# MartinMikkelsen/TensorTrainNumerics.jl

Hardware: AMD Instinct MI355X
Metric: TT cores/sec for QTT Laplacian apply+round, d=30 rank-64 (higher is better)
Workload: dtype f64

## Files before the change

### tensortrainnumerics.jl_amd/csrc/ttn_dense_kernels.h

```cpp
#pragma once
#include "ttn_wg_prims.h"
#include "ttn_wg_gemm.h"
#include "ttn_wg_lq.h"
#include "ttn_wg_jacobi.h"
#include "ttn_wg_chol.h"

struct CompressArgs {
    TTDev tt;
    long long max_bond;
    double truncerr;
    int sweeps;
    int k_single;
    int k_first, k_last;
    double* scratch;
    long long scratch_stride;
    int pmax, qmax;
    double* sv_out;
    int sv_steps;
    int* status;
    int* sweep_stats;
    int fast;
    int fused;
    TTODev op;
    TTDev x;
    int rank_rule;
    int fused_first_real;
    int* next_train;
};

#define COMPRESS_LDS_X_DOUBLES (128 * 128)
#define COMPRESS_LDS_BYTES ((GEMM_LDS_TOTAL + 32 + 2 * QR_NB * QR_NB + QR_NB + 8 + 8 + 128) * sizeof(double))
#define FAST_KAPPA_MAX 128.0
#define FAST_KAPPA_POLISH 32768.0
#define FAST_POLISH_DROP 1.0e-12
#define FAST_DIAG_TOL 2.0e-12
#define FAST_CHECK_TOL 2.0e-11

struct BondCtx {
    double *ldsX, *red, *Ts, *Ss, *taus, *scal, *nrm2;
    int* iflag;
    double *M, *M2, *Vb, *Wb, *Us, *Xg, *sig, *sigs, *Ga, *Gb, *Cc, *T1, *T2, *T3;
    int* perm;
};

#define CHOLQR_PIVOT_MAX 1.0e11
#define CHOLQR_ORTH_MAX 1.0e-3
#define CHOLQR_CHECK_TOL 1.0e-9

__device__ __noinline__ double wg_img_load(double* img, int row_off, const double* src, int p, double* red) {
    img = unip(img); src = unip(src); p = uni32(p); row_off = uni32(row_off); red = unip(red);
    lds_f64* X = (lds_f64*)img;
    double dev = 0.0;
    wg_batched<8>((long long)p * p, [&](long long e) { const int ei = (int)e; return src[ei % p + 128 * (ei / p)]; },
                  [&](long long e, double v) {
                      const int ei = (int)e, i = ei % p, j = ei / p;
                      X[row_off + i + 128 * j] = v;
                      dev = fmax(dev, fabs(v - ((i == j) ? 1.0 : 0.0)));
                  });
    return unif64(wg_max(dev, red));
}

__device__ __noinline__ void wg_trsm_lower_cols(int p, int q, const double* img, const double* M, long long ldm, double s_, double* Q, long long ldq) {
    p = uni32(p); q = uni32(q); img = unip(img); M = unip(M); Q = unip(Q); ldm = uni64(ldm); ldq = uni64(ldq); s_ = unif64(s_);
    const lds_f64* L = (const lds_f64*)img;
    gmem_f64* Mg = (gmem_f64*)M;
    gmem_wf64* Qg = (gmem_wf64*)Q;
    for (int c = threadIdx.x; c < q; c += TTN_WG) {
        for (int i0 = 0; i0 < p; i0 += 16) {
            const int nb = (p - i0 < 16) ? p - i0 : 16;
            double v[16];
#pragma unroll
            for (int ii = 0; ii < 16; ++ii) v[ii] = Mg[(long long)(i0 + (ii < nb ? ii : 0)) * ldm + c];
#pragma unroll
            for (int ii = 0; ii < 16; ++ii) v[ii] *= s_;
            for (int j0 = 0; j0 < i0; j0 += 16) {
                double qv[16];
#pragma unroll
                for (int jj = 0; jj < 16; ++jj) qv[jj] = Qg[(long long)(j0 + jj) * ldq + c];
#pragma unroll
                for (int jj = 0; jj < 16; ++jj)
#pragma unroll
                    for (int ii = 0; ii < 16; ++ii) v[ii] = fma(-L[(j0 + jj) * 128 + i0 + ii], qv[jj], v[ii]);
            }
#pragma unroll
            for (int k = 0; k < 16; ++k) {
                if (k < nb) {
                    v[k] = v[k] / L[(i0 + k) * 128 + i0 + k];
#pragma unroll
                    for (int ii = k + 1; ii < 16; ++ii) v[ii] = fma(-L[(i0 + k) * 128 + i0 + ii], v[k], v[ii]);
                }
            }
#pragma unroll
            for (int ii = 0; ii < 16; ++ii) if (ii < nb) Qg[(long long)(i0 + ii) * ldq + c] = v[ii];
        }
    }
    __syncthreads();
}

__device__ __noinline__ void wg_tril_mul_lds(int p, double* img) {
    p = uni32(p); img = unip(img);
    lds_f64* X = (lds_f64*)img;
    constexpr int NE = (64 * 64 + TTN_WG - 1) / TTN_WG;
    double acc[NE];
#pragma unroll
    for (int u = 0; u < NE; ++u) {
        const int e = threadIdx.x + u * TTN_WG, i = e % p, j = e / p;
        double a = 0.0;
        if (e < p * p && i >= j)
            for (int k = j; k <= i; ++k) a = fma(X[64 + i + 128 * k], X[k + 128 * j], a);
        acc[u] = a;
    }
    __syncthreads();
    for (int e = threadIdx.x; e < p * 128; e += TTN_WG) X[e] = 0.0;
    __syncthreads();
#pragma unroll
    for (int u = 0; u < NE; ++u) {
        const int e = threadIdx.x + u * TTN_WG, i = e % p, j = e / p;
        if (e < p * p && i >= j) X[i + 128 * j] = acc[u];
    }
    __syncthreads();
}

__device__ __noinline__ void wg_scale_image(const double* X, int ldx, int x_in_lds, const double* sigs, const int* perm, View Lo, double* Us, int p, int r,
                                            double s0, double aneg, int mode, double* tab) {
    X = unip(X); ldx = uni32(ldx); x_in_lds = uni32(x_in_lds); sigs = unip(sigs); perm = unip(perm); Lo = uniView(Lo); Us = unip(Us);
    p = uni32(p); r = uni32(r); s0 = unif64(s0); aneg = unif64(aneg); mode = uni32(mode); tab = unip(tab);
    lds_f64* f1 = (lds_f64*)tab; lds_f64* f2 = f1 + 128;
    lds_i32* pj = (lds_i32*)(f2 + 128); lds_i32* coff = pj + 128; lds_i32* roff = coff + 128;
    const int tid = threadIdx.x, lane = tid & 63, wave = tid >> 6;
    const double sq0 = sqrt(s0);
    for (int j = tid; j < r; j += TTN_WG) {
        const double sj = sigs[j];
        const bool keep = (sj > 0.0) && (sj * sj > aneg);
        double a, b_;
        if (mode == 0) { const double rs = sqrt(sj); a = sq0 / rs; b_ = sq0 / (sj * rs); }
        else if (mode == 1) { a = 1.0 / sj; b_ = s0 / sj; }
        else { a = s0; b_ = 1.0 / (sj * sj); }
        f1[j] = keep ? a : 0.0; f2[j] = keep ? b_ : 0.0;
        pj[j] = perm[j]; coff[j] = (int)ix(Lo.c, j);
    }
    for (int i = tid; i < p; i += TTN_WG) roff[i] = (int)ix(Lo.r, i);
    __syncthreads();
    gmem_wf64* Lg = (gmem_wf64*)Lo.p;
    gmem_wf64* Ug = (gmem_wf64*)Us;
    for (int j = wave; j < r; j += TTN_NWAVES) {
        const double a = f1[j], b_ = f2[j];
        const int c = pj[j], co = coff[j];
        for (int row = lane; row < p; row += 64) {
            const double xv = x_in_lds ? ((const lds_f64*)X)[c * ldx + row] : X[(long long)c * ldx + row];
            Lg[roff[row] + co] = xv * a;
            Ug[j * p + row] = xv * b_;
        }
    }
    __syncthreads();
}

__device__ __noinline__ double wg_check_diag_tab(const double* sigs, const double* D, int ldd, int r, double s0, double* tab, double* red) {
    sigs = unip(sigs); D = unip(D); ldd = uni32(ldd); r = uni32(r); s0 = unif64(s0); tab = unip(tab); red = unip(red);
    lds_f64* t = (lds_f64*)tab; lds_f64* ref = t + 128;
    const int tid = threadIdx.x, lane = tid & 63, wave = tid >> 6;
    for (int i = tid; i < r; i += TTN_WG) { const double si = sigs[i]; t[i] = 1.0 / sqrt(s0 * si); ref[i] = si * s0; }
    __syncthreads();
    gmem_f64* Dg = (gmem_f64*)D;
    double worst = 0.0;
    for (int j = wave; j < r; j += TTN_NWAVES) {
        const double tj = t[j];
        for (int i = lane; i < r; i += 64) {
            const double dv = Dg[i + ldd * j];
            const double dev = fabs(dv - ((i == j) ? ref[i] : 0.0)) * (t[i] * tj);
            worst = fmax(worst, dev);
        }
    }
    return unif64(wg_max(worst, red));
}

__device__ __noinline__ double wg_check_diag_tab2(const double* sigs, const double* D1, const double* D2, int ldd, int r, double s0, double* tab, double* red) {
    sigs = unip(sigs); D1 = unip(D1); D2 = unip(D2); ldd = uni32(ldd); r = uni32(r); s0 = unif64(s0); tab = unip(tab); red = unip(red);
    lds_f64* t = (lds_f64*)tab; lds_f64* ref = t + 128;
    const int tid = threadIdx.x, lane = tid & 63, wave = tid >> 6;
    for (int i = tid; i < r; i += TTN_WG) { const double si = sigs[i]; t[i] = 1.0 / sqrt(s0 * si); ref[i] = si * s0; }
    __syncthreads();
    gmem_f64* D1g = (gmem_f64*)D1; gmem_f64* D2g = (gmem_f64*)D2;
    double worst = 0.0;
    for (int j = wave; j < r; j += TTN_NWAVES) {
        const double tj = t[j];
        for (int i = lane; i < r; i += 64) {
            const double d1 = D1g[i + ldd * j], d2 = D2g[i + ldd * j];
            const double rf = (i == j) ? ref[i] : 0.0, sc = t[i] * tj;
            worst = fmax(worst, fmax(fabs(d1 - rf) * sc, fabs(d2 - rf) * sc));
        }
    }
    return unif64(wg_max(worst, red));
}

__device__ __noinline__ double wg_diag_test_t3(const double* Ga, const double* Gb, double* T3, double* tab, double* red) {
    Ga = unip(Ga); Gb = unip(Gb); T3 = unip(T3); tab = unip(tab); red = unip(red);
    lds_f64* sd = (lds_f64*)tab; lds_f64* isd = sd + 64;
    const int tid = threadIdx.x, lane = tid & 63, wave = tid >> 6;
    gmem_f64* Gag = (gmem_f64*)Ga; gmem_f64* Gbg = (gmem_f64*)Gb; gmem_wf64* Tg = (gmem_wf64*)T3;
    for (int i = tid; i < 64; i += TTN_WG) { const double d = Gag[i * 129]; const double sq = (d > 0.0) ? sqrt(d) : 0.0; sd[i] = sq; isd[i] = (d > 0.0) ? 1.0 / sq : -1.0; }
    __syncthreads();
    double w = 0.0;
    const double si = sd[lane], ii = isd[lane];
    constexpr int NJ = 64 / TTN_NWAVES;
    double ga[NJ], gb[NJ];
#pragma unroll
    for (int u = 0; u < NJ; ++u) { const int j = wave + TTN_NWAVES * u; ga[u] = Gag[lane + 128 * j]; gb[u] = Gbg[lane + 128 * j]; }
#pragma unroll
    for (int u = 0; u < NJ; ++u) {
        const int j = wave + TTN_NWAVES * u;
        const double ij = isd[j];
        if (lane != j) w = fmax(w, (ii > 0.0 && ij > 0.0) ? fabs(ga[u]) * (ii * ij) : 1.0);
        Tg[lane + 128 * j] = si * gb[u] * sd[j];
    }
    w = unif64(wg_max(w, red));
    return w;
}

__device__ __noinline__ void wg_scale_t12_diag(const double* img, const double* sigs, const int* perm, const double* Ga, double* T1, double* T2, int rk,
                                               double fa, double fb, double* tab) {
    img = unip(img); sigs = unip(sigs); perm = unip(perm); Ga = unip(Ga); T1 = unip(T1); T2 = unip(T2); rk = uni32(rk); fa = unif64(fa); fb = unif64(fb); tab = unip(tab);
    lds_f64* c1 = (lds_f64*)tab; lds_f64* c2 = c1 + 64; lds_f64* sd = c2 + 64; lds_f64* isd = sd + 64;
    lds_i32* pj = (lds_i32*)(isd + 64);
    const lds_f64* X = (const lds_f64*)img;
    const int tid = threadIdx.x, lane = tid & 63, wave = tid >> 6;
    for (int j = tid; j < 64; j += TTN_WG) {
        const double d = sqrt(Ga[j * 129]); sd[j] = d; isd[j] = 1.0 / d;
        if (j < rk) { const double sj = sigs[j], rs = sqrt(sj); c1[j] = fa / rs; c2[j] = fb / (sj * rs); pj[j] = perm[j]; }
    }
    __syncthreads();
    gmem_wf64* T1g = (gmem_wf64*)T1; gmem_wf64* T2g = (gmem_wf64*)T2;
    const double sdr = sd[lane], isdr = isd[lane];
    for (int j = wave; j < rk; j += TTN_NWAVES) {
        const double xv = X[pj[j] * 128 + lane];
        T1g[j * 128 + lane] = xv * (c1[j] * isdr);
        T2g[j * 128 + lane] = xv * (sdr * c2[j]);
    }
    __syncthreads();
}

__device__ int wg_svd_cols(const CompressArgs& P, const BondCtx& S, int pj, double* X, int ldx, bool in_lds, int mlen = 0) {
    const int tid = threadIdx.x, lane = tid & 63, wave = tid >> 6, nwaves = TTN_WG >> 6;
    const int nsw = (in_lds && mlen) ? wg_jacobi_lds128(mlen, pj, X, S.nrm2, S.iflag, S.red, S.scal)
                  : in_lds ? wg_jacobi_lds128(pj, pj, X, S.nrm2, S.iflag, S.red, S.scal)
#if TTN_LDS_COLS < 128
                  : (pj <= 128) ? wg_jacobi_blocked128(pj, pj, X, ldx, S.ldsX, S.nrm2, S.iflag, S.red, S.scal)
#endif
                  : (pj <= 256) ? wg_jacobi_blocked256(pj, pj, X, ldx, S.ldsX, S.nrm2, S.iflag, S.red, S.scal)
                                : wg_jacobi_cols(pj, pj, X, ldx, S.iflag, S.red, S.scal);
    for (int c = wave; c < pj; c += nwaves) {
        double a = 0.0;
        for (int r = lane; r < (mlen ? mlen : pj); r += 64) { const double v = X[(long long)c * ldx + r]; a = fma(v, v, a); }
        a = wave_sum(a);
        if (lane == 0) S.sig[c] = sqrt(a);
    }
    __syncthreads();
    for (int c = tid; c < pj; c += TTN_WG) {
        const double sc = S.sig[c];
        int pos = 0;
        for (int j = 0; j < pj; ++j) { const double sj = S.sig[j]; pos += (sj > sc) || (sj == sc && j < c); }
        S.perm[pos] = c;
        S.sigs[pos] = sc;
    }
    __syncthreads();
    return nsw;
}

__device__ __forceinline__ int wg_rank_rule_core(int rank_rule, double truncerr, long long max_bond, const double* sigs, int* iflag, int ns, int plen, double s0) {
    if (threadIdx.x == 0) {
        int r = plen;
        if (rank_rule == 1) {
            if (truncerr > 0.0) {
                r = 0;
                const double thr = truncerr * (sigs[0] * s0);
                for (int i = 0; i < ns; ++i) r += (sigs[i] * s0 > thr) ? 1 : 0;
                if (r < 1) r = 1;
            }
        } else if (truncerr > 0.0) {
            double n2 = 0.0;
            for (int i = 0; i < ns; ++i) { const double s = sigs[i] * s0; n2 = fma(s, s, n2); }
            const double nrm = sqrt(n2);
            double cum = 0.0;
            for (int i = plen; i >= 1; --i) {
                const double s = (i <= ns) ? sigs[i - 1] * s0 : 0.0;
                cum = fma(s, s, cum);
                if (sqrt(cum) > truncerr * nrm) { r = i; break; }
            }
        }
        if ((long long)r > max_bond) r = (int)max_bond;
        iflag[1] = r;
// ... 565 lines not shown
    const int n1 = io.n1, n2 = io.n2;
    const int Dl = io.Dl, rm = io.rm, Dr = io.Dr;
    const int mr = n1 * Dl, mc = n2 * Dr;
    double* ck = io.ck;
    double* ck1 = io.ck1;
    const View Am = mkview(ck, Idx{Dl, (long long)n1, 1}, plain((long long)n1 * Dl));
    const View Bm = mkview(ck1, plain(n2), Idx{n2, 1, (long long)n2 * rm});
    const bool wide = mr <= mc;
    const int p = wide ? mr : mc, q = wide ? mc : mr;
    const View Ap = wide ? Am : tview(Bm);
    const View Bp = wide ? Bm : tview(Am);

    BondCtx S;
    S.ldsX = lds;
    S.red = lds + GEMM_LDS_TOTAL;
    S.Ts = S.red + 32;
    S.Ss = S.Ts + QR_NB * QR_NB;
    S.taus = S.Ss + QR_NB * QR_NB;
    S.scal = S.taus + QR_NB;
    S.iflag = reinterpret_cast<int*>(S.scal + 8);
    S.nrm2 = S.scal + 16;
    double* scr = P.scratch + (long long)blockIdx.x * P.scratch_stride;
    const long long pq = (long long)P.pmax * P.qmax;
    S.M = scr;
    S.M2 = S.M + pq;
    S.Vb = S.M2 + pq;
    S.Wb = S.Vb + (long long)QR_NB * P.qmax;
    S.Us = S.Wb + (long long)P.pmax * QR_NB;
    S.Xg = S.Us + (long long)P.pmax * P.pmax;
    S.sig = S.Xg + (long long)P.pmax * P.pmax;
    S.sigs = S.sig + P.pmax;
    S.perm = reinterpret_cast<int*>(S.sigs + P.pmax);
    S.Ga = S.sigs + 2 * P.pmax;
    S.Gb = S.Ga + 128 * 128;
    S.Cc = S.Gb + 128 * 128;
    S.T1 = S.Cc + 128 * 128;
    S.T2 = S.T1 + 128 * 128;
    S.T3 = S.T2 + 128 * 128;
    if (pq >= 3 * 128 * 128) {
        S.Ga = S.M2; S.Gb = S.M2 + 128 * 128; S.T2 = S.M2 + 2 * 128 * 128;
    }

    bool virt_live = false;
    if (virt) {
        if (wide && rm >= p) virt_live = true;
        else wg_materialize_core(P, b, k + 1);
    }

    const View Lfv = mkview(ck, Idx{Dl, (long long)n1, 1}, plain((long long)n1 * Dl));
    int nsw_total = 0;
    bool done = false;

    if (SWAP == 0 && P.fast && rm < p && rm <= TTN_LDS_COLS && rm >= 2) {
        double sa = 0.0, sb = 0.0;
        sa = wg_absmax(ck, (long long)n1 * Dl * rm, S.red);
        sb = wg_absmax(ck1, (long long)n2 * rm * Dr, S.red);
        bool ok = (sa > 0.0) && (sb > 0.0);
        const double sA = wide ? sa : sb, sB = wide ? sb : sa;
        const double s0 = sA * sB;
        const View Gav = mkview(S.Ga, plain(1), plain(128));
        const View Gbv = mkview(S.Gb, plain(1), plain(128));
        const View Ccv = mkview(S.Cc, plain(1), plain(128));
        bool diagA = false;
        if (ok) {
            wg_syrk2(rm, p, tview(Ap), Gav, 1.0 / (sA * sA), rm, q, Bp, Gbv, 1.0 / (sB * sB), lds);
            if (rm == 64 && !(P.fast & 4) && !(P.fast & 8)) {
                const double wmax = wg_diag_test_t3(S.Ga, S.Gb, S.T3, S.Ss, S.red);
                diagA = wmax <= FAST_DIAG_TOL;
            }
            if (diagA) {
            } else if (rm <= TTN_LDS_COLS / 2) {
                for (int e = tid; e < rm * 128; e += TTN_WG) if ((e & 127) < rm) { S.ldsX[e] = S.Ga[e]; S.ldsX[TTN_LDS_IMG / 2 + e] = S.Gb[e]; }
                __syncthreads();
                ok = wg_chol2_lds128(rm, S.ldsX, S.Ts, S.iflag, S.scal + 1) == 0;
                for (int e = tid; e < rm * 128; e += TTN_WG) if ((e & 127) < rm) { S.Ga[e] = S.ldsX[e]; S.Gb[e] = S.ldsX[TTN_LDS_IMG / 2 + e]; }
                __syncthreads();
            } else {
                for (int e = tid; e < rm * 128; e += TTN_WG) if ((e & 127) < rm) S.ldsX[e] = S.Ga[e];
                __syncthreads();
                ok = wg_chol_lds128(rm, S.ldsX, S.red, S.iflag, S.scal + 1) == 0;
                for (int e = tid; e < rm * 128; e += TTN_WG) if ((e & 127) < rm) S.Ga[e] = S.ldsX[e];
                __syncthreads();
                if (ok) {
                    for (int e = tid; e < rm * 128; e += TTN_WG) if ((e & 127) < rm) S.ldsX[e] = S.Gb[e];
                    __syncthreads();
                    ok = wg_chol_lds128(rm, S.ldsX, S.red, S.iflag, S.scal + 1) == 0;
                    for (int e = tid; e < rm * 128; e += TTN_WG) if ((e & 127) < rm) S.Gb[e] = S.ldsX[e];
                    __syncthreads();
                }
            }
        }
        int r = 0, rk = 0;
        if (ok) {
            int nsw = 1;
            if (diagA) {
                ok = wg_eig64(S.T3, 128, S.T2, 64, 64, S.sigs, lds, reinterpret_cast<int*>(S.Ts), S.Ts + 64) == 0;
                for (int j = tid; j < 64; j += TTN_WG) S.perm[j] = j;
                if (tid == 0) S.scal[0] = 64.0 * DBL_EPSILON * DBL_EPSILON * S.sigs[0] * S.sigs[0];
                __syncthreads();
            } else {
            wg_gemm(rm, rm, rm, tview(Gav), Gbv, Ccv, 1.0, 0.0, lds);
            if (rm == 64 && !(P.fast & 4)) {
                wg_gemm(64, 64, 64, Ccv, tview(Ccv), mkview(S.T3, plain(1), plain(128)), 1.0, 0.0, lds);
                ok = wg_eig64(S.T3, 128, S.T2, 64, 64, S.sigs, lds, reinterpret_cast<int*>(S.Ts), S.Ts + 64) == 0;
                for (int j = tid; j < 64; j += TTN_WG) S.perm[j] = j;
                if (tid == 0) S.scal[0] = 64.0 * DBL_EPSILON * DBL_EPSILON * S.sigs[0] * S.sigs[0];
                __syncthreads();
            } else {
                for (int e = tid; e < rm * 128; e += TTN_WG) { const int c = e >> 7, r_ = e & 127; S.ldsX[e] = (r_ < rm) ? S.Cc[c * 128 + r_] : 0.0; }
// ... 88 lines not shown
        for (int attempt = (SWAP == 0 && P.fast && need_lq && (eig_ok || cholqr_ok || (x_in_lds && !lq_in_lds)) && p >= 2) ? 1 : 2; attempt <= 2 && !done; ++attempt) {
            bool ok = true;
            bool use_eig = false;
            bool cholqr = false;
            double gram_trace = 0.0;
            X = (x_in_lds || attempt == 1) ? S.ldsX : S.Xg;
            ldx = (x_in_lds || attempt == 1) ? 128 : p;
            if (attempt == 1) {
                wg_syrk(p, q, Mv, mkview(S.Ga, plain(1), plain(128)), inv_s0 * inv_s0, lds);
                use_eig = eig_ok;
                if (use_eig) {
                    if (p > 64 && p < 128) {
                        for (int e = tid; e < 128 * 128; e += TTN_WG)
                            if ((e & 127) >= p || (e >> 7) >= p) S.Ga[e] = 0.0;
                        __syncthreads();
                    }
                    const int r0 = (int)P.max_bond;
                    const int nev = (P.truncerr > 0.0 || (P.sv_out && step < P.sv_steps)) ? p : r0;
                    { double t_ = 0.0; for (int i = tid; i < p; i += TTN_WG) t_ += S.Ga[i * 129]; gram_trace = unif64(wg_sum(t_, S.red)); }
                    ok = ((p == 64) ? wg_eig64(S.Ga, 128, S.Gb, r0, nev, S.sigs, lds, reinterpret_cast<int*>(S.Ts), S.Ts + 64)
                                    : wg_eig128(S.Ga, S.Gb, r0, nev, S.sigs, lds, reinterpret_cast<int*>(S.Ts), S.Ts + 64)) == 0;
                    for (int j = tid; j < p; j += TTN_WG) { S.perm[j] = j; if (j >= nev) S.sigs[j] = 0.0; }
                    if (tid == 0) S.scal[0] = (double)p * DBL_EPSILON * DBL_EPSILON * S.sigs[0] * S.sigs[0];
                    __syncthreads();
                } else {
                wg_img_load(S.ldsX, 0, S.Ga, p, S.red);
                ok = wg_chol_lds128(p, S.ldsX, S.red, S.iflag, S.scal + 1) == 0;
                if (ok && (P.truncerr > 0.0 || (long long)p <= P.max_bond)) {
                    if (cholqr_ok) { if (unif64(S.scal[1]) <= CHOLQR_PIVOT_MAX) cholqr = true; else ok = false; }
                    else if (unif64(S.scal[1]) > FAST_KAPPA_MAX * FAST_KAPPA_MAX) ok = false;
                }
                if (cholqr) {
                    for (int e = tid; e < p * p; e += TTN_WG) { const int i = e % p, j = e / p; S.T1[i + 128 * j] = S.ldsX[i + 128 * j]; }
                    wg_trsm_lower_cols(p, q, S.ldsX, S.M, q, inv_s0, S.M2, q);
                    const View Q1v = mkview(S.M2, plain(q), plain(1));
                    wg_syrk(p, q, Q1v, mkview(S.Cc, plain(1), plain(128)), 1.0, lds);
                    const double dev = wg_img_load(S.ldsX, 0, S.Cc, p, S.red);
                    ok = dev <= CHOLQR_ORTH_MAX && wg_chol_lds128(p, S.ldsX, S.red, S.iflag, S.scal + 1) == 0;
                    if (ok) {
                        wg_img_load(S.ldsX, 64, S.T1, p, S.red);
                        wg_tril_mul_lds(p, S.ldsX);
                    }
                }
                for (int e = tid; e < p * 128; e += TTN_WG) if ((e & 127) >= p) S.ldsX[e] = 0.0;
                __syncthreads();
                }
            } else {
                if (need_lq) {
                    wg_copy_scale(S.M2, S.M, (long long)p * q, inv_s0);
                    __syncthreads();
                    wg_lq_blocked(p, q, S.M2, q, S.Vb, S.Wb, nullptr, nullptr, lds, S.Ts, S.Ss, S.taus, S.red);
                }
                const double* Lsrc = need_lq ? S.M2 : S.M;
                if (need_lq && x_in_lds) {
                    const int lane_ = tid & 63, wave_ = tid >> 6;
                    for (int c = wave_; c < p; c += TTN_NWAVES) {
                        double a = 0.0;
                        for (int r_ = c + lane_; r_ < p; r_ += 64) { const double v = Lsrc[(long long)r_ * q + c]; a = fma(v, v, a); }
                        a = wave_sum(a);
                        if (lane_ == 0) S.sig[c] = a;
                    }
                    __syncthreads();
                    for (int c = tid; c < p; c += TTN_WG) {
                        const double sc = S.sig[c];
                        int pos = 0;
                        for (int j = 0; j < p; ++j) { const double sj = S.sig[j]; pos += (sj > sc) || (sj == sc && j < c); }
                        S.perm[c] = pos;
                    }
                    __syncthreads();
                }
                const bool presort = need_lq && x_in_lds;
                for (int e = tid; e < p * ldx; e += TTN_WG) {
                    const int r_ = e % ldx, c = e / ldx;
                    const double v = (r_ < p) ? Lsrc[(long long)r_ * q + c] * (need_lq ? 1.0 : inv_s0) : 0.0;
                    const int cd = presort ? S.perm[c] : c;
                    X[(long long)cd * ldx + r_] = (need_lq && c > r_) ? 0.0 : v;
                }
                __syncthreads();
            }
            int nsw = 0;
            if (ok && !(attempt == 1 && use_eig)) {
                nsw = uni32(wg_svd_cols(P, S, p, X, ldx, x_in_lds));
                nsw_total += (nsw < 0 ? -nsw : nsw);
                if (attempt == 1) ok = nsw > 0;
                else if (nsw < 0 && tid == 0) ttn_set_status(&P.status[b], TTN_ST_JACOBI);
            }
            if (!ok) continue;
            const int r = wg_rank_rule(P, S, p, p, s0);
            if (SWAP != 0 && r > io.cap) {
                if (tid == 0) { ttn_set_status(&P.status[b], TTN_ST_RANK_OVERFLOW); *io.rank_out = -1; }
                __syncthreads();
                done = true;
                continue;
            }
            if (attempt == 1 && !cholqr) {
                const int rl = (P.truncerr > 0.0) ? p : r;
                if (__builtin_expect(!((S.sigs[rl - 1] * FAST_KAPPA_MAX >= S.sigs[0]) && (S.sigs[rl - 1] * S.sigs[rl - 1] > S.scal[0])), 0)) {
                    bool polish = use_eig && SWAP == 0 && !(P.fast & 16) && P.truncerr == 0.0 && q <= 128 && r <= 64 && r >= 2 &&
                                  (S.sigs[r - 1] * FAST_KAPPA_POLISH >= S.sigs[0]) && (S.sigs[r - 1] * S.sigs[r - 1] > S.scal[0]);
                    if (polish) {
                        double kept = 0.0;
                        for (int j = tid; j < r; j += TTN_WG) kept = fma(S.sigs[j], S.sigs[j], kept);
                        kept = unif64(wg_sum(kept, S.red));
                        polish = (gram_trace - kept) <= FAST_POLISH_DROP * gram_trace;
                    }
                    if (!polish) continue;
                    const double aneg0 = S.scal[0];
                    for (int e = tid; e < p * r; e += TTN_WG) {
                        const int row = e % p, j = e / p;
                        const double sj = S.sigs[j], xv = X[(long long)S.perm[j] * ldx + row];
                        S.Us[(long long)j * p + row] = ((sj > 0.0) && (sj * sj > aneg0)) ? xv / sj : 0.0;
                    }
                    __syncthreads();
                    wg_gemm_ra(r, q, p, mkview(S.Us, plain(p), plain(1)), Mv, mkview(S.M2, plain(q), plain(1)), inv_s0, lds);
                    for (int e = tid; e < r * 128; e += TTN_WG) { const int c = e & 127, j = e >> 7; S.ldsX[e] = (c < q) ? S.M2[(long long)j * q + c] : 0.0; }
                    __syncthreads();
                    const int nsp = uni32(wg_svd_cols(P, S, r, S.ldsX, 128, true, q));
                    nsw_total += (nsp < 0 ? -nsp : nsp);
                    if (nsp <= 0) continue;
                    const View Rfv = mkview(ck1, plain(n2), Idx{n2, 1, (long long)n2 * r});
                    const View Lo = wide ? Lfv : tview(Rfv);
                    const View Ro = wide ? Rfv : tview(Lfv);
                    const double sq0 = sqrt(s0), aneg = S.scal[0];
                    for (int e = tid; e < r * q; e += TTN_WG) {
                        const int col = e % q, j = e / q;
                        const double sj = S.sigs[j], xv = S.ldsX[S.perm[j] * 128 + col];
                        const bool keep = (sj > 0.0) && (sj * sj > aneg);
                        Ro.p[ix(Ro.r, j) + ix(Ro.c, col)] = keep ? xv * (sq0 / sqrt(sj)) : 0.0;
                        S.M2[(long long)j * q + col] = keep ? xv * (sq0 / (sj * sqrt(sj))) : 0.0;
                    }
                    __syncthreads();
                    wg_gemm(p, r, q, Mv, mkview(S.M2, plain(1), plain(q)), Lo, inv_s0, 0.0, lds);
                    if (P.sv_out && step < P.sv_steps) {
                        double* so = P.sv_out + ((long long)b * P.sv_steps + step) * P.pmax;
                        for (int i = tid; i < P.pmax; i += TTN_WG) so[i] = (i < p) ? S.sigs[i] * s0 : -1.0;
                    }
                    if (tid == 0) *io.rank_out = r;
                    __syncthreads();
                    done = true;
                    continue;
                }
            }
            if (attempt == 2 && P.sv_out && step < P.sv_steps) {
                double* so = P.sv_out + ((long long)b * P.sv_steps + step) * P.pmax;
                for (int i = tid; i < P.pmax; i += TTN_WG) so[i] = (i < p) ? S.sigs[i] * s0 : -1.0;
            }
            const View Rfv = mkview(ck1, plain(n2), Idx{n2, 1, (long long)n2 * r});
            const View Lo = wide ? Lfv : tview(Rfv);
            const View Ro = wide ? Rfv : tview(Lfv);
            const double sq0 = sqrt(s0);
            const double aneg = S.scal[0];
            if (p <= 128 && r <= 128) {
                wg_scale_image(X, ldx, (x_in_lds || attempt == 1) ? 1 : 0, S.sigs, S.perm, Lo, S.Us, p, r, s0, aneg, (SWAP == 0) ? 0 : (wide ? 1 : 2), S.Ts);
            } else {
            for (int e = tid; e < p * r; e += TTN_WG) {
                const int row = e % p, j = e / p;
                const double sj = S.sigs[j];
                const double xv = X[(long long)S.perm[j] * ldx + row];
                const bool keep = (sj > 0.0) && (sj * sj > aneg);
                double lf, us;
                if (SWAP == 0) { lf = keep ? xv * (sq0 / sqrt(sj)) : 0.0; us = keep ? xv * (sq0 / (sj * sqrt(sj))) : 0.0; }
                else if (wide) { lf = keep ? xv / sj : 0.0; us = keep ? xv * (s0 / sj) : 0.0; }
                else { lf = keep ? xv * s0 : 0.0; us = keep ? xv / (sj * sj) : 0.0; }
                Lo.p[ix(Lo.r, row) + ix(Lo.c, j)] = lf;
                S.Us[(long long)j * p + row] = us;
            }
            }
            __syncthreads();
            wg_gemm_ra(r, q, p, mkview(S.Us, plain(p), plain(1)), Mv, Ro, inv_s0, lds);
// ... 86 lines not shown
```

### tensortrainnumerics.jl_amd/csrc/ttn_wg_prims.h

```cpp
#pragma once
#include "ttn_common.h"
#include <float.h>

#define TTN_SETPRIO_GEMM() __builtin_amdgcn_s_setprio(0)
#define TTN_SETPRIO_BASE() __builtin_amdgcn_s_setprio(TTN_PRIO_BASE)

#if TTN_WG == 512
#define TTN_LDS_IMG (64 * 128)
#else
#define TTN_LDS_IMG (128 * 128)
#endif
#define TTN_LDS_COLS (TTN_LDS_IMG / 128)

template <int CTRL>
__device__ inline double dpp_mov_f64(double v) {
    union { double d; int i[2]; } a, r;
    a.d = v;
    r.i[0] = __builtin_amdgcn_update_dpp(0, a.i[0], CTRL, 0xF, 0xF, true);
    r.i[1] = __builtin_amdgcn_update_dpp(0, a.i[1], CTRL, 0xF, 0xF, true);
    return r.d;
}
__device__ inline double row16_sum(double v) {
    v += dpp_mov_f64<0xB1>(v);
    v += dpp_mov_f64<0x4E>(v);
// ... 17 lines not shown
    for (int r = 0; r < 4; ++r) {
        union { double d; int i[2]; } w;
        w.i[0] = __builtin_amdgcn_readlane(u.i[0], 16 * r);
        w.i[1] = __builtin_amdgcn_readlane(u.i[1], 16 * r);
        t += w.d;
    }
    return t;
}
__device__ inline double wave64_max_fast(double v) {
    v = row16_max(v);
    union { double d; int i[2]; } u;
    u.d = v;
    double t = -1.7976931348623157e308;
#pragma unroll
    for (int r = 0; r < 4; ++r) {
        union { double d; int i[2]; } w;
        w.i[0] = __builtin_amdgcn_readlane(u.i[0], 16 * r);
        w.i[1] = __builtin_amdgcn_readlane(u.i[1], 16 * r);
        t = fmax(t, w.d);
    }
    return t;
}
__device__ inline double wave_sum(double v) { return wave64_sum_fast(v); }
__device__ inline double wave_max(double v) { return wave64_max_fast(v); }
__device__ inline double wg_sum(double v, double* red) {
    v = wave_sum(v);
    const int w = threadIdx.x >> 6, l = threadIdx.x & 63, nw = blockDim.x >> 6;
    __syncthreads();
    if (l == 0) red[w] = v;
    __syncthreads();
    double t = (l < nw) ? red[l] : 0.0;
    __syncthreads();
    t = wave_sum(t);
    return t;
}
__device__ inline double wg_max(double v, double* red) {
    v = wave_max(v);
    const int w = threadIdx.x >> 6, l = threadIdx.x & 63, nw = blockDim.x >> 6;
    __syncthreads();
    if (l == 0) red[w] = v;
    __syncthreads();
    double t = (l < nw) ? red[l] : 0.0;
    __syncthreads();
    t = wave_max(t);
    return t;
}

typedef double mfma_acc_t __attribute__((ext_vector_type(4)));
typedef __attribute__((address_space(3))) double lds_f64;
typedef __attribute__((address_space(3))) long long lds_i64;
typedef __attribute__((address_space(3))) int lds_i32;
typedef const __attribute__((address_space(1))) double gmem_f64;
typedef __attribute__((address_space(1))) double gmem_wf64;

__device__ inline int uni32(int v) { return __builtin_amdgcn_readfirstlane(v); }
__device__ inline long long uni64(long long v) {
    const int lo = __builtin_amdgcn_readfirstlane((int)(v & 0xffffffffLL));
    const int hi = __builtin_amdgcn_readfirstlane((int)(v >> 32));
    return ((long long)hi << 32) | (unsigned int)lo;
}
template <typename PT> __device__ inline PT* unip(PT* q_) { return (PT*)uni64((long long)q_); }
__device__ inline double unif64(double v) { union { double d; long long i; } u; u.d = v; u.i = uni64(u.i); return u.d; }
__device__ inline Idx uniIdx(const Idx& d) { return Idx{uni32(d.q), uni64(d.lo), uni64(d.hi)}; }
__device__ inline View uniView(const View& v) { return View{(double*)uni64((long long)v.p), uniIdx(v.r), uniIdx(v.c)}; }

template <int U, typename LoadF, typename UseF>
__device__ __forceinline__ void wg_batched(long long n, LoadF load, UseF use) {
    for (long long e0 = threadIdx.x; e0 < n; e0 += (long long)TTN_WG * U) {
        decltype(load(0LL)) v[U];
#pragma unroll
        for (int u = 0; u < U; ++u) { const long long e = e0 + (long long)u * TTN_WG; v[u] = load(e < n ? e : e0); }
#pragma unroll
        for (int u = 0; u < U; ++u) { const long long e = e0 + (long long)u * TTN_WG; if (e < n) use(e, v[u]); }
    }
}
__device__ __noinline__ void wg_copy_scale(double* dst, const double* src, long long n, double s_) {
    dst = unip(dst); src = unip(src); n = uni64(n); s_ = unif64(s_);
    wg_batched<8>(n, [&](long long e) { return src[e]; }, [&](long long e, double v) { dst[e] = v * s_; });
}
__device__ __noinline__ double wg_absmax(const double* src, long long n, double* red) {
    src = unip(src); n = uni64(n); red = unip(red);
    double m_ = 0.0;
    wg_batched<8>(n, [&](long long e) { return src[e]; }, [&](long long, double v) { m_ = fmax(m_, fabs(v)); });
    return unif64(wg_max(m_, red));
}
__device__ __noinline__ void wg_copy_to_view(View dst, const double* src, int rows, int cols, long long rs, long long cs, int lim, int col_lim) {
    dst = uniView(dst); src = unip(src); rows = uni32(rows); cols = uni32(cols); rs = uni64(rs); cs = uni64(cs); lim = uni32(lim); col_lim = uni32(col_lim);
    const bool row_fast = rs <= cs;
    const int fast = row_fast ? rows : cols;
    wg_batched<8>((long long)rows * cols,
                  [&](long long e) {
                      const int ei = (int)e, lo = ei % fast, hi = ei / fast;
                      const int i = row_fast ? lo : hi, j = row_fast ? hi : lo;
                      return ((col_lim ? j : i) < lim) ? src[i * rs + j * cs] : 0.0;
                  },
                  [&](long long e, double v) {
                      const int ei = (int)e, lo = ei % fast, hi = ei / fast;
                      const int i = row_fast ? lo : hi, j = row_fast ? hi : lo;
                      dst.p[ix(dst.r, i) + ix(dst.c, j)] = v;
                  });
}

__device__ inline double fast_rcp(double x) {
    double y = __builtin_amdgcn_rcp(x);
    y = fma(fma(-x, y, 1.0), y, y);
    return y;
}
__device__ inline double fast_rsqrt2(double w) {
    double y = __builtin_amdgcn_rsq(w);
    double h = 0.5 * w;
    y = y * fma(-h * y, y, 1.5);
    y = y * fma(-h * y, y, 1.5);
    return y;
}
```

Before: 654,400.

## Use explicit address-space loads, fuse absmax pair, and outline image-building helpers

Casts global and LDS pointers to explicit address spaces so the compiler can emit global and ds instructions instead of flat accesses. It adds an idempotent batched loop that writes clamped duplicate elements rather than branching, and fuses the two absmax reductions into one pass. It also moves the inline LQ-image, polish and row-to-image loops into noinline batched helpers, and rewrites copy_to_view with incremental index arithmetic to avoid per-element division. The risks are subtle indexing bugs in the new incremental index code and extra register pressure.

Result: no change. 656,100, median of 3 (+0.3%).

```diff
diff --git a/tensortrainnumerics.jl_amd/csrc/ttn_dense_kernels.h b/tensortrainnumerics.jl_amd/csrc/ttn_dense_kernels.h
--- a/tensortrainnumerics.jl_amd/csrc/ttn_dense_kernels.h
+++ b/tensortrainnumerics.jl_amd/csrc/ttn_dense_kernels.h
@@ -50,14 +50,15 @@
 __device__ __noinline__ double wg_img_load(double* img, int row_off, const double* src, int p, double* red) {
     img = unip(img); src = unip(src); p = uni32(p); row_off = uni32(row_off); red = unip(red);
     lds_f64* X = (lds_f64*)img;
+    gmem_f64* sg = (gmem_f64*)src;
     double dev = 0.0;
-    wg_batched<8>((long long)p * p, [&](long long e) { const int ei = (int)e; return src[ei % p + 128 * (ei / p)]; },
+    wg_batched_idem<8>((long long)p * p, [&](long long e) { const int ei = (int)e; return sg[ei % p + 128 * (ei / p)]; },
                   [&](long long e, double v) {
                       const int ei = (int)e, i = ei % p, j = ei / p;
                       X[row_off + i + 128 * j] = v;
                       dev = fmax(dev, fabs(v - ((i == j) ? 1.0 : 0.0)));
                   });
-    return unif64(wg_max(dev, red));
+    return unif64(wg_max_lds(dev, (lds_f64*)red));
 }
 
 __device__ __noinline__ void wg_trsm_lower_cols(int p, int q, const double* img, const double* M, long long ldm, double s_, double* Q, long long ldq) {
@@ -130,14 +131,14 @@
     const int tid = threadIdx.x, lane = tid & 63, wave = tid >> 6;
     const double sq0 = sqrt(s0);
     for (int j = tid; j < r; j += TTN_WG) {
-        const double sj = sigs[j];
+        const double sj = ((gmem_f64*)sigs)[j];
         const bool keep = (sj > 0.0) && (sj * sj > aneg);
         double a, b_;
         if (mode == 0) { const double rs = sqrt(sj); a = sq0 / rs; b_ = sq0 / (sj * rs); }
         else if (mode == 1) { a = 1.0 / sj; b_ = s0 / sj; }
         else { a = s0; b_ = 1.0 / (sj * sj); }
         f1[j] = keep ? a : 0.0; f2[j] = keep ? b_ : 0.0;
-        pj[j] = perm[j]; coff[j] = (int)ix(Lo.c, j);
+        pj[j] = ((gmem_i32*)perm)[j]; coff[j] = (int)ix(Lo.c, j);
     }
     for (int i = tid; i < p; i += TTN_WG) roff[i] = (int)ix(Lo.r, i);
     __syncthreads();
@@ -147,7 +148,7 @@
         const double a = f1[j], b_ = f2[j];
         const int c = pj[j], co = coff[j];
         for (int row = lane; row < p; row += 64) {
-            const double xv = x_in_lds ? ((const lds_f64*)X)[c * ldx + row] : X[(long long)c * ldx + row];
+            const double xv = x_in_lds ? ((const lds_f64*)X)[c * ldx + row] : ((gmem_f64*)X)[(long long)c * ldx + row];
             Lg[roff[row] + co] = xv * a;
             Ug[j * p + row] = xv * b_;
         }
@@ -159,7 +160,7 @@
     sigs = unip(sigs); D = unip(D); ldd = uni32(ldd); r = uni32(r); s0 = unif64(s0); tab = unip(tab); red = unip(red);
     lds_f64* t = (lds_f64*)tab; lds_f64* ref = t + 128;
     const int tid = threadIdx.x, lane = tid & 63, wave = tid >> 6;
-    for (int i = tid; i < r; i += TTN_WG) { const double si = sigs[i]; t[i] = 1.0 / sqrt(s0 * si); ref[i] = si * s0; }
+    for (int i = tid; i < r; i += TTN_WG) { const double si = ((gmem_f64*)sigs)[i]; t[i] = 1.0 / sqrt(s0 * si); ref[i] = si * s0; }
     __syncthreads();
     gmem_f64* Dg = (gmem_f64*)D;
     double worst = 0.0;
@@ -171,14 +172,14 @@
             worst = fmax(worst, dev);
         }
     }
-    return unif64(wg_max(worst, red));
+    return unif64(wg_max_lds(worst, (lds_f64*)red));
 }
 
 __device__ __noinline__ double wg_check_diag_tab2(const double* sigs, const double* D1, const double* D2, int ldd, int r, double s0, double* tab, double* red) {
     sigs = unip(sigs); D1 = unip(D1); D2 = unip(D2); ldd = uni32(ldd); r = uni32(r); s0 = unif64(s0); tab = unip(tab); red = unip(red);
     lds_f64* t = (lds_f64*)tab; lds_f64* ref = t + 128;
     const int tid = threadIdx.x, lane = tid & 63, wave = tid >> 6;
-    for (int i = tid; i < r; i += TTN_WG) { const double si = sigs[i]; t[i] = 1.0 / sqrt(s0 * si); ref[i] = si * s0; }
+    for (int i = tid; i < r; i += TTN_WG) { const double si = ((gmem_f64*)sigs)[i]; t[i] = 1.0 / sqrt(s0 * si); ref[i] = si * s0; }
     __syncthreads();
     gmem_f64* D1g = (gmem_f64*)D1; gmem_f64* D2g = (gmem_f64*)D2;
     double worst = 0.0;
@@ -190,7 +191,7 @@
             worst = fmax(worst, fmax(fabs(d1 - rf) * sc, fabs(d2 - rf) * sc));
         }
     }
-    return unif64(wg_max(worst, red));
+    return unif64(wg_max_lds(worst, (lds_f64*)red));
 }
 
 __device__ __noinline__ double wg_diag_test_t3(const double* Ga, const double* Gb, double* T3, double* tab, double* red) {
@@ -213,7 +214,7 @@
         if (lane != j) w = fmax(w, (ii > 0.0 && ij > 0.0) ? fabs(ga[u]) * (ii * ij) : 1.0);
         Tg[lane + 128 * j] = si * gb[u] * sd[j];
     }
-    w = unif64(wg_max(w, red));
+    w = unif64(wg_max_lds(w, (lds_f64*)red));
     return w;
 }
 
@@ -225,8 +226,8 @@
     const lds_f64* X = (const lds_f64*)img;
     const int tid = threadIdx.x, lane = tid & 63, wave = tid >> 6;
     for (int j = tid; j < 64; j += TTN_WG) {
-        const double d = sqrt(Ga[j * 129]); sd[j] = d; isd[j] = 1.0 / d;
-        if (j < rk) { const double sj = sigs[j], rs = sqrt(sj); c1[j] = fa / rs; c2[j] = fb / (sj * rs); pj[j] = perm[j]; }
+        const double d = sqrt(((gmem_f64*)Ga)[j * 129]); sd[j] = d; isd[j] = 1.0 / d;
+        if (j < rk) { const double sj = ((gmem_f64*)sigs)[j], rs = sqrt(sj); c1[j] = fa / rs; c2[j] = fb / (sj * rs); pj[j] = ((gmem_i32*)perm)[j]; }
     }
     __syncthreads();
     gmem_wf64* T1g = (gmem_wf64*)T1; gmem_wf64* T2g = (gmem_wf64*)T2;
@@ -236,6 +237,90 @@
         T1g[j * 128 + lane] = xv * (c1[j] * isdr);
         T2g[j * 128 + lane] = xv * (sdr * c2[j]);
     }
+    __syncthreads();
+}
+
+__device__ __noinline__ void wg_lq_image(const double* Lsrc, int q, int p, int need_lq, double inv_s0, double* X, int ldx, int x_in_lds, double* tab) {
+    Lsrc = unip(Lsrc); q = uni32(q); p = uni32(p); need_lq = uni32(need_lq); inv_s0 = unif64(inv_s0); X = unip(X); ldx = uni32(ldx);
+    x_in_lds = uni32(x_in_lds); tab = unip(tab);
+    gmem_f64* Lg = (gmem_f64*)Lsrc;
+    const int tid = threadIdx.x, lane = tid & 63, wave = tid >> 6;
+    if (need_lq && x_in_lds) {
+        lds_f64* Xl = (lds_f64*)X;
+        lds_f64* nrm = (lds_f64*)tab; lds_i32* cpos = (lds_i32*)(nrm + 128);
+        constexpr int NE = TTN_LDS_IMG / TTN_WG;
+        double v[NE];
+#pragma unroll
+        for (int u = 0; u < NE; ++u) {
+            const int e = tid + u * TTN_WG, r_ = e & 127, c = e >> 7;
+            v[u] = Lg[(r_ < p && c <= r_) ? (long long)r_ * q + c : 0];
+        }
+#pragma unroll
+        for (int u = 0; u < NE; ++u) {
+            const int e = tid + u * TTN_WG, r_ = e & 127, c = e >> 7;
+            v[u] = (r_ < p && c <= r_) ? v[u] * 1.0 : 0.0;
+            Xl[e] = v[u];
+        }
+        __syncthreads();
+        for (int c = wave; c < p; c += TTN_NWAVES) {
+            double a = 0.0;
+            for (int r_ = c + lane; r_ < p; r_ += 64) { const double w = Xl[c * 128 + r_]; a = fma(w, w, a); }
+            a = wave_sum(a);
+            if (lane == 0) nrm[c] = a;
+        }
+        __syncthreads();
+        for (int c = tid; c < p; c += TTN_WG) {
+            const double sc = nrm[c];
+            int pos = 0;
+            for (int j = 0; j < p; ++j) { const double sj = nrm[j]; pos += (sj > sc) || (sj == sc && j < c); }
+            cpos[c] = pos;
+        }
+        __syncthreads();
+#pragma unroll
+        for (int u = 0; u < NE; ++u) {
+            const int e = tid + u * TTN_WG, r_ = e & 127, c = e >> 7;
+            Xl[((c < p) ? cpos[c] : c) * 128 + r_] = v[u];
+        }
+    } else {
+        const double f = need_lq ? 1.0 : inv_s0;
+        const int n = p * ldx;
+        auto load = [&](long long e) {
+            const int ei = (int)e, r_ = ei % ldx, c = ei / ldx;
+            return Lg[(r_ < p && !(need_lq && c > r_)) ? (long long)r_ * q + c : 0];
+        };
+        auto value = [&](long long e, double w) {
+            const int ei = (int)e, r_ = ei % ldx, c = ei / ldx;
+            return (r_ < p && !(need_lq && c > r_)) ? w * f : 0.0;
+        };
+        if (x_in_lds) { lds_f64* Xl = (lds_f64*)X; wg_batched_idem<8>(n, load, [&](long long e, double w) { Xl[e] = value(e, w); }); }
+        else { gmem_wf64* Xg = (gmem_wf64*)X; wg_batched_idem<8>(n, load, [&](long long e, double w) { Xg[e] = value(e, w); }); }
+    }
+    __syncthreads();
+}
+
+__device__ __noinline__ void wg_polish_us(const double* img, const double* sigs, const int* perm, double* Us, int p, int r, double aneg, double* tab) {
+    img = unip(img); sigs = unip(sigs); perm = unip(perm); Us = unip(Us); p = uni32(p); r = uni32(r); aneg = unif64(aneg); tab = unip(tab);
+    const lds_f64* X = (const lds_f64*)img;
+    lds_f64* sg = (lds_f64*)tab; lds_i32* pj = (lds_i32*)(sg + 64); lds_i32* kp = pj + 64;
+    const int tid = threadIdx.x, lane = tid & 63, wave = tid >> 6;
+    for (int j = tid; j < r; j += TTN_WG) {
+        const double sj = ((gmem_f64*)sigs)[j];
+        sg[j] = sj; kp[j] = ((sj > 0.0) && (sj * sj > aneg)) ? 1 : 0; pj[j] = ((gmem_i32*)perm)[j];
+    }
+    __syncthreads();
+    gmem_wf64* Ug = (gmem_wf64*)Us;
+    for (int j = wave; j < r; j += TTN_NWAVES) {
+        const double sj = sg[j];
+        const int c = pj[j], keep = kp[j];
+        for (int row = lane; row < p; row += 64) Ug[j * p + row] = keep ? X[c * 128 + row] / sj : 0.0;
+    }
+    __syncthreads();
+}
+__device__ __noinline__ void wg_rows_to_image(double* img, const double* src, int r, int q) {
+    img = unip(img); src = unip(src); r = uni32(r); q = uni32(q);
+    lds_f64* X = (lds_f64*)img; gmem_f64* sg = (gmem_f64*)src;
+    wg_batched_idem<8>((long long)r * 128, [&](long long e) { const int ei = (int)e, c = ei & 127, j = ei >> 7; return sg[(c < q) ? j * q + c : 0]; },
+                  [&](long long e, double w) { const int ei = (int)e; X[ei] = ((ei & 127) < q) ? w : 0.0; });
     __syncthreads();
 }
 
@@ -907,9 +992,8 @@
     bool done = false;
 
     if (SWAP == 0 && P.fast && rm < p && rm <= TTN_LDS_COLS && rm >= 2) {
-        double sa = 0.0, sb = 0.0;
-        sa = wg_absmax(ck, (long long)n1 * Dl * rm, S.red);
-        sb = wg_absmax(ck1, (long long)n2 * rm * Dr, S.red);
+        const AbsMax2 sab = wg_absmax2(ck, (long long)n1 * Dl * rm, ck1, (long long)n2 * rm * Dr, S.red);
+        const double sa = sab.a, sb = sab.b;
         bool ok = (sa > 0.0) && (sb > 0.0);
         const double sA = wide ? sa : sb, sB = wide ? sb : sa;
         const double s0 = sA * sB;
@@ -1104,31 +1188,7 @@
                     wg_lq_blocked(p, q, S.M2, q, S.Vb, S.Wb, nullptr, nullptr, lds, S.Ts, S.Ss, S.taus, S.red);
                 }
                 const double* Lsrc = need_lq ? S.M2 : S.M;
-                if (need_lq && x_in_lds) {
-                    const int lane_ = tid & 63, wave_ = tid >> 6;
-                    for (int c = wave_; c < p; c += TTN_NWAVES) {
-                        double a = 0.0;
-                        for (int r_ = c + lane_; r_ < p; r_ += 64) { const double v = Lsrc[(long long)r_ * q + c]; a = fma(v, v, a); }
-                        a = wave_sum(a);
-                        if (lane_ == 0) S.sig[c] = a;
-                    }
-                    __syncthreads();
-                    for (int c = tid; c < p; c += TTN_WG) {
-                        const double sc = S.sig[c];
-                        int pos = 0;
-                        for (int j = 0; j < p; ++j) { const double sj = S.sig[j]; pos += (sj > sc) || (sj == sc && j < c); }
-                        S.perm[c] = pos;
-                    }
-                    __syncthreads();
-                }
-                const bool presort = need_lq && x_in_lds;
-                for (int e = tid; e < p * ldx; e += TTN_WG) {
-                    const int r_ = e % ldx, c = e / ldx;
-                    const double v = (r_ < p) ? Lsrc[(long long)r_ * q + c] * (need_lq ? 1.0 : inv_s0) : 0.0;
-                    const int cd = presort ? S.perm[c] : c;
-                    X[(long long)cd * ldx + r_] = (need_lq && c > r_) ? 0.0 : v;
-                }
-                __syncthreads();
+                wg_lq_image(Lsrc, q, p, need_lq ? 1 : 0, inv_s0, X, ldx, x_in_lds ? 1 : 0, S.Ts);
             }
             int nsw = 0;
             if (ok && !(attempt == 1 && use_eig)) {
@@ -1157,16 +1217,9 @@
                         polish = (gram_trace - kept) <= FAST_POLISH_DROP * gram_trace;
                     }
                     if (!polish) continue;
-                    const double aneg0 = S.scal[0];
-                    for (int e = tid; e < p * r; e += TTN_WG) {
-                        const int row = e % p, j = e / p;
-                        const double sj = S.sigs[j], xv = X[(long long)S.perm[j] * ldx + row];
-                        S.Us[(long long)j * p + row] = ((sj > 0.0) && (sj * sj > aneg0)) ? xv / sj : 0.0;
-                    }
-                    __syncthreads();
+                    wg_polish_us(S.ldsX, S.sigs, S.perm, S.Us, p, r, S.scal[0], S.Ts);
                     wg_gemm_ra(r, q, p, mkview(S.Us, plain(p), plain(1)), Mv, mkview(S.M2, plain(q), plain(1)), inv_s0, lds);
-                    for (int e = tid; e < r * 128; e += TTN_WG) { const int c = e & 127, j = e >> 7; S.ldsX[e] = (c < q) ? S.M2[(long long)j * q + c] : 0.0; }
-                    __syncthreads();
+                    wg_rows_to_image(S.ldsX, S.M2, r, q);
                     const int nsp = uni32(wg_svd_cols(P, S, r, S.ldsX, 128, true, q));
                     nsw_total += (nsp < 0 ? -nsp : nsp);
                     if (nsp <= 0) continue;
diff --git a/tensortrainnumerics.jl_amd/csrc/ttn_wg_prims.h b/tensortrainnumerics.jl_amd/csrc/ttn_wg_prims.h
--- a/tensortrainnumerics.jl_amd/csrc/ttn_wg_prims.h
+++ b/tensortrainnumerics.jl_amd/csrc/ttn_wg_prims.h
@@ -93,6 +93,18 @@
 typedef __attribute__((address_space(3))) int lds_i32;
 typedef const __attribute__((address_space(1))) double gmem_f64;
 typedef __attribute__((address_space(1))) double gmem_wf64;
+typedef const __attribute__((address_space(1))) int gmem_i32;
+__device__ inline double wg_max_lds(double v, lds_f64* red) {
+    v = wave_max(v);
+    const int w = threadIdx.x >> 6, l = threadIdx.x & 63, nw = blockDim.x >> 6;
+    __syncthreads();
+    if (l == 0) red[w] = v;
+    __syncthreads();
+    double t = (l < nw) ? red[l] : 0.0;
+    __syncthreads();
+    t = wave_max(t);
+    return t;
+}
 
 __device__ inline int uni32(int v) { return __builtin_amdgcn_readfirstlane(v); }
 __device__ inline long long uni64(long long v) {
@@ -115,31 +127,89 @@
         for (int u = 0; u < U; ++u) { const long long e = e0 + (long long)u * TTN_WG; if (e < n) use(e, v[u]); }
     }
 }
+template <int U, typename LoadF, typename UseF>
+__device__ __forceinline__ void wg_batched_idem(long long n, LoadF load, UseF use) {
+    for (long long e0 = threadIdx.x; e0 < n; e0 += (long long)TTN_WG * U) {
+        decltype(load(0LL)) v[U];
+#pragma unroll
+        for (int u = 0; u < U; ++u) { const long long e = e0 + (long long)u * TTN_WG; v[u] = load(e < n ? e : e0); }
+#pragma unroll
+        for (int u = 0; u < U; ++u) { const long long e = e0 + (long long)u * TTN_WG; use(e < n ? e : e0, v[u]); }
+    }
+}
 __device__ __noinline__ void wg_copy_scale(double* dst, const double* src, long long n, double s_) {
     dst = unip(dst); src = unip(src); n = uni64(n); s_ = unif64(s_);
-    wg_batched<8>(n, [&](long long e) { return src[e]; }, [&](long long e, double v) { dst[e] = v * s_; });
-}
-__device__ __noinline__ double wg_absmax(const double* src, long long n, double* red) {
-    src = unip(src); n = uni64(n); red = unip(red);
-    double m_ = 0.0;
-    wg_batched<8>(n, [&](long long e) { return src[e]; }, [&](long long, double v) { m_ = fmax(m_, fabs(v)); });
-    return unif64(wg_max(m_, red));
+    gmem_wf64* dg = (gmem_wf64*)dst; gmem_f64* sg = (gmem_f64*)src;
+    wg_batched_idem<8>(n, [&](long long e) { return sg[e]; }, [&](long long e, double v) { dg[e] = v * s_; });
+}
+struct AbsMax2 { double a, b; };
+__device__ __noinline__ AbsMax2 wg_absmax2(const double* a, long long na, const double* b, long long nb, double* red) {
+    a = unip(a); na = uni64(na); b = unip(b); nb = uni64(nb); red = unip(red);
+    gmem_f64* ag = (gmem_f64*)a; gmem_f64* bg = (gmem_f64*)b;
+    double ma = 0.0, mb = 0.0;
+    const long long n = na > nb ? na : nb;
+    for (long long e0 = threadIdx.x; e0 < n; e0 += (long long)TTN_WG * 8) {
+        double va[8], vb[8];
+#pragma unroll
+        for (int u = 0; u < 8; ++u) { const long long e = e0 + (long long)u * TTN_WG; va[u] = ag[e < na ? e : 0]; vb[u] = bg[e < nb ? e : 0]; }
+#pragma unroll
+        for (int u = 0; u < 8; ++u) { ma = fmax(ma, fabs(va[u])); mb = fmax(mb, fabs(vb[u])); }
+    }
+    ma = wave_max(ma); mb = wave_max(mb);
+    const int w = threadIdx.x >> 6, l = threadIdx.x & 63;
+    lds_f64* rl = (lds_f64*)red;
+    __syncthreads();
+    if (l == 0) { rl[w] = ma; rl[16 + w] = mb; }
+    __syncthreads();
+    double ta = (l < TTN_NWAVES) ? rl[l] : 0.0, tb = (l < TTN_NWAVES) ? rl[16 + l] : 0.0;
+    __syncthreads();
+    AbsMax2 out;
+    out.a = unif64(wave_max(ta)); out.b = unif64(wave_max(tb));
+    return out;
 }
 __device__ __noinline__ void wg_copy_to_view(View dst, const double* src, int rows, int cols, long long rs, long long cs, int lim, int col_lim) {
     dst = uniView(dst); src = unip(src); rows = uni32(rows); cols = uni32(cols); rs = uni64(rs); cs = uni64(cs); lim = uni32(lim); col_lim = uni32(col_lim);
     const bool row_fast = rs <= cs;
     const int fast = row_fast ? rows : cols;
-    wg_batched<8>((long long)rows * cols,
-                  [&](long long e) {
-                      const int ei = (int)e, lo = ei % fast, hi = ei / fast;
-                      const int i = row_fast ? lo : hi, j = row_fast ? hi : lo;
-                      return ((col_lim ? j : i) < lim) ? src[i * rs + j * cs] : 0.0;
-                  },
-                  [&](long long e, double v) {
-                      const int ei = (int)e, lo = ei % fast, hi = ei / fast;
-                      const int i = row_fast ? lo : hi, j = row_fast ? hi : lo;
-                      dst.p[ix(dst.r, i) + ix(dst.c, j)] = v;
-                  });
+    const int n = rows * cols;
+    const Idx fi = row_fast ? dst.r : dst.c, si = row_fast ? dst.c : dst.r;
+    const int fstr = (int)(row_fast ? rs : cs), sstr = (int)(row_fast ? cs : rs);
+    const bool lim_slow = (col_lim != 0) == row_fast;
+    const int fq = fi.q ? fi.q : 0x7fffffff, sq = si.q ? si.q : 0x7fffffff;
+    const long long flo = fi.lo, fhi = fi.q ? fi.hi : 0, slo = si.lo, shi = si.q ? si.hi : 0;
+    const int df = TTN_WG % fast, ds = TTN_WG / fast;
+    const int da = df % fq, db = df / fq, wa = fast % fq, wb = fast / fq, dc = ds % sq, dd = ds / sq;
+    gmem_f64* sg = (gmem_f64*)src; gmem_wf64* dg = (gmem_wf64*)dst.p;
+    for (int e0 = threadIdx.x; e0 < n; e0 += TTN_WG * 8) {
+        int f = e0 % fast, s_ = e0 / fast;
+        int a = f % fq, b = f / fq, c = s_ % sq, d = s_ / sq;
+        int so[8];
+        long long dofs[8];
+        double v[8];
+        unsigned keep = 0;
+#pragma unroll
+        for (int u = 0; u < 8; ++u) {
+            if (e0 + u * TTN_WG < n) {
+                const bool k_ = (lim_slow ? s_ : f) < lim;
+                so[u] = k_ ? f * fstr + s_ * sstr : 0;
+                dofs[u] = a * flo + b * fhi + c * slo + d * shi;
+                keep |= (unsigned)k_ << u;
+            } else {
+                so[u] = so[0]; dofs[u] = dofs[0];
+                keep |= (keep & 1u) << u;
+            }
+            f += df; a += da; b += db;
+            if (a >= fq) { a -= fq; b += 1; }
+            int carry = 0;
+            if (f >= fast) { f -= fast; a -= wa; b -= wb; if (a < 0) { a += fq; b -= 1; } carry = 1; }
+            s_ += ds + carry; c += dc + carry; d += dd;
+            if (c >= sq) { c -= sq; d += 1; }
+        }
+#pragma unroll
+        for (int u = 0; u < 8; ++u) v[u] = sg[so[u]];
+#pragma unroll
+        for (int u = 0; u < 8; ++u) dg[dofs[u]] = ((keep >> u) & 1u) ? v[u] : 0.0;
+    }
 }
 
 __device__ inline double fast_rcp(double x) {
```
